# m4drat/wtf

Measured on AMD Instinct MI355X. Metric: execs/sec + emulated instr/s per node (tlv_server, HEVD) at 1/2/4/8 GPUs, higher is better.
Workload: dtype u64

## Files before the change

wtf_amd/csrc/engine.hip:

```cpp
#include <hip/hip_runtime.h>
#include <hipcub/device/device_radix_sort.hpp>

#include <algorithm>
#include <cstddef>
#include <cstdio>
#include <cstdlib>
#include <cstring>
#include <new>
#include <vector>

#include "engine_run.h"
#include "engine_kernels.h"

using namespace wtfgpu_dev;

#define HIPCHK(x)                                                                        \
  do {                                                                                   \
    hipError_t e_ = (x);                                                                 \
    if (e_ != hipSuccess) {                                                              \
      fprintf(stderr, "wtfgpu: %s failed: %s (%s:%d)\n", #x, hipGetErrorString(e_), __FILE__, \
              __LINE__);                                                                 \
      return WTFGPU_ERR_HIP;                                                             \
    }                                                                                    \
  } while (0)
// ... 992 lines not shown
static int set_status_list(wtfgpu_ctx *c, const uint32_t *lanes, uint32_t n, uint32_t status, const uint8_t *skip) {
  if (!c || !c->d_status || (n && !lanes)) return WTFGPU_ERR_INVALID;
  if (n == 0) return WTFGPU_OK;
  for (u32 i = 0; i < n; i++)
    if (lanes[i] >= c->P.nlanes) return WTFGPU_ERR_INVALID;
  HIPCHK(hipSetDevice(c->device));
  const u64 o_skip = ((u64)n * 4 + 255) & ~255ull;
  u8 *st = ring_put(c, nullptr, o_skip + n);
  if (!st || ensure_scratch(c, o_skip + n)) return WTFGPU_ERR_OOM;
  memcpy(st, lanes, (u64)n * 4);
  if (skip) memcpy(st + o_skip, skip, n);
  HIPCHK(hipMemcpyAsync(c->d_scratch, st, skip ? o_skip + n : (u64)n * 4, hipMemcpyHostToDevice, c->stream));
  k_set_status<<<(n + 255) / 256, 256, 0, c->stream>>>(c->P, (const u32 *)c->d_scratch, n, status,
                                                      skip ? c->d_scratch + o_skip : nullptr);
  HIPCHK(hipGetLastError());
  return WTFGPU_OK;
}

int wtfgpu_resume(wtfgpu_ctx *c, const uint32_t *lanes, uint32_t n, const uint8_t *skip_bp) {
  std::vector<u8> zeros;
  if (!skip_bp) {
    zeros.assign(n, 0);
    skip_bp = zeros.data();
  }
  return set_status_list(c, lanes, n, WTFGPU_RUNNING, skip_bp);
}

int wtfgpu_stop(wtfgpu_ctx *c, const uint32_t *lanes, uint32_t n, uint32_t status) {
  return set_status_list(c, lanes, n, status, nullptr);
}

static int regroup_buffers(wtfgpu_ctx *c) {
  if (c->d_rkeys) return WTFGPU_OK;
  const u64 N = c->P.nlanes;
  if (!c->d_perm && dalloc(&c->d_perm, N)) return WTFGPU_ERR_OOM;
  if (dalloc(&c->d_rkeys, N) || dalloc(&c->d_rkeys2, N) || dalloc(&c->d_rlanes, N)) return WTFGPU_ERR_OOM;
  size_t bytes = 0;
  HIPCHK(hipcub::DeviceRadixSort::SortPairs(nullptr, bytes, c->d_rkeys, c->d_rkeys2, c->d_rlanes, c->d_perm, (int)N, 0,
                                            24, c->stream));
  HIPCHK(hipMalloc(&c->d_rtemp, bytes));
  c->rtemp_bytes = bytes;
  return WTFGPU_OK;
}

static Dev run_params(wtfgpu_ctx *c, bool regroup) {
  Dev Q = c->P;
  Q.perm = regroup ? c->d_perm : nullptr;
  Q.stat = c->d_stat;
  const char *w = getenv("WTFGPU_WARM");
  if (!(w && atoi(w) == 0)) {
    const u32 need = (u32)((c->P.nlanes + c->P.lpw - 1) / c->P.lpw);
    if (c->d_warm && c->warm_n < need) {
      (void)hipDeviceSynchronize();
      (void)hipFree(c->d_warm);
      c->d_warm = nullptr;
    }
    if (!c->d_warm) {
      c->warm_n = need;
      const u64 bytes = UC_IMAGE_BYTES * need * UC_QUEUES;
      if (hipMalloc((void **)&c->d_warm, bytes) != hipSuccess) {
        c->d_warm = nullptr;
      } else if (hipMemset(c->d_warm, 0xff, bytes) != hipSuccess || hipDeviceSynchronize() != hipSuccess) {
        (void)hipFree(c->d_warm);
        c->d_warm = nullptr;
      }
    }
    Q.warm = c->d_warm ? c->d_warm + (u64)(c->cur_queue % UC_QUEUES) * UC_IMAGE_BYTES * c->warm_n : nullptr;
    Q.warm_n = c->warm_n;
  } else {
    Q.warm = nullptr;
  }
  return Q;
}

static u64 regroup_now(wtfgpu_ctx *c, u32 count) {
  c->rg_used[c->cur_queue & 1] = 2;
  if (!c->regroup_steps || count < 2 * c->P.lpw) return 0;
  if (!c->regroup_auto) return c->regroup_steps;
  static constexpr double kMargin = 1.1;
  static constexpr u64 kProbe = 32;
  const u64 i = c->rg_runs++;
  bool on;
  if (c->lps_sched[1] == 0) on = true;
  else if (c->lps_sched[0] == 0) on = false;
  else {
    on = c->lps_sched[1] > kMargin * c->lps_sched[0];
    if (i % kProbe == kProbe - 1) on = !on;
  }
  c->rg_used[c->cur_queue & 1] = on;
  return on ? c->regroup_steps : 0;
}
static u64 regroup_now_timed(wtfgpu_ctx *c, u32 count, int &used) {
  used = 2;
  if (!c->regroup_steps || count < 2 * c->P.lpw) return 0;
  if (!c->regroup_auto) return c->regroup_steps;
  static constexpr u64 kProbe = 32;
  const u64 i = c->rg_sync_runs++;
  bool on;
  if (c->nspi_sched[1] == 0) on = true;
  else if (c->nspi_sched[0] == 0) on = false;
  else {
    on = c->nspi_sched[1] < c->nspi_sched[0];
    if (i % kProbe == kProbe - 1) on = !on;
  }
  used = on;
  return on ? c->regroup_steps : 0;
}
static void regroup_observe_timed(wtfgpu_ctx *c, int used, double ms, u64 retired) {
  if (used > 1 || retired < 4096) return;
  const double v = ms * 1e6 / (double)retired;
  double &e = c->nspi_sched[used];
  e = e == 0 ? v : 0.75 * e + 0.25 * v;
}
static void regroup_observe(wtfgpu_ctx *c, u64 group_steps, u64 retired) {
  const u8 used = c->rg_used[c->cur_queue & 1];
  if (used > 1 || group_steps < 64) return;
  const double lps = (double)retired / (double)group_steps;
  double &e = c->lps_sched[used];
  e = e == 0 ? lps : 0.75 * e + 0.25 * lps;
}

static int launch_chunk(wtfgpu_ctx *c, const Dev &Q, u32 first, u32 count, u64 steps, bool regroup) {
  const u32 hwaves = (count + c->P.lpw - 1) / c->P.lpw;
  if (regroup) {
    HIPCHK(hipMemsetAsync(c->d_stat + 2, 0, 16, c->stream));
    k_regroup_keys<<<(count + 255) / 256, 256, 0, c->stream>>>(Q, first, count, c->d_rkeys, c->d_rlanes);
    HIPCHK(hipGetLastError());
    size_t bytes = c->rtemp_bytes;
    HIPCHK(hipcub::DeviceRadixSort::SortPairs(c->d_rtemp, bytes, c->d_rkeys, c->d_rkeys2, c->d_rlanes,
                                              c->d_perm + first, (int)count, 0, 24, c->stream));
  }
  k_run<<<(hwaves + 3) / 4, 256, 0, c->stream>>>(Q, first, count, steps);
  HIPCHK(hipGetLastError());
  return WTFGPU_OK;
}

static void print_stamps(const u64 *s) {
#ifdef WTFGPU_STAMPS
  if (s[0])
    fprintf(stderr,
            "wtfgpu stamps (cycles per wave-step, %llu steps): fast loop %.0f, slow: xlate+fill %.0f, coverage %.0f, "
            "exec %.0f, cross-page %.0f; slow steps: miss %llu, codepage %llu, ucmiss %llu, other %llu; "
            "fast lookup %.0f, fast exec %.0f, bp %.0f\n",
            (unsigned long long)s[0], (double)s[4] / s[0], (double)s[6] / s[0], (double)s[7] / s[0],
            (double)s[5] / s[0], (double)s[9] / s[0], (unsigned long long)s[12], (unsigned long long)s[13],
            (unsigned long long)s[14], (unsigned long long)s[15], (double)s[10] / s[0], (double)s[11] / s[0], (double)s[8] / s[0]);
  fprintf(stderr, "wtfgpu stamps generic ops:");
  for (int k = 0; k < 512; k++)
    if (s[16 + k]) fprintf(stderr, " %d:%llu", k, (unsigned long long)s[16 + k]);
  fprintf(stderr, "\n");
  fprintf(stderr, "wtfgpu stamps bp_apply cycles by kind:");
  for (int k = 0; k < 8; k++) fprintf(stderr, " %d:%llu", k, (unsigned long long)s[528 + k]);
  fprintf(stderr, "\n");
#else
  (void)s;
#endif
}

int wtfgpu_run(wtfgpu_ctx *c, uint32_t first, uint32_t count, uint64_t max_steps, wtfgpu_run_stats_t *stats) {
  if (!lanes_ok(c, first, count) || (first % c->P.lpw)) return WTFGPU_ERR_INVALID;
  if (!c->P.pool) return WTFGPU_ERR_STATE;
  if (c->async_launches) return WTFGPU_ERR_STATE;
  HIPCHK(hipSetDevice(c->device));
  wtfgpu_run_stats_t st{};
  u64 chunk = 1ull << 20;
  const bool to_end = max_steps >= (1ull << 32);
  int used_timed = 2;
  const u64 regroup = to_end ? regroup_now_timed(c, count, used_timed) : regroup_now(c, count);
  if (regroup) {
    chunk = regroup;
    if (int rc = regroup_buffers(c)) return rc;
  }
  const Dev Q = run_params(c, regroup != 0);
  const u32 group = regroup ? (u32)std::max<u64>(1, 4096 / regroup) : 1;
  u64 done = 0;
  float ms_total = 0;
  for (;;) {
    HIPCHK(hipMemsetAsync(c->d_stat, 0, STAT_N * 8, c->stream));
    HIPCHK(hipEventRecord(c->ev0, c->stream));
    u32 k = 0;
    for (; k < group && done < max_steps; k++) {
      const u64 steps = std::min<u64>(chunk, max_steps - done);
      if (int rc = launch_chunk(c, Q, first, count, steps, regroup != 0)) return rc;
      done += steps;
    }
    HIPCHK(hipEventRecord(c->ev1, c->stream));
    u64 s[STAT_N];
    HIPCHK(hipMemcpyAsync(s, c->d_stat, sizeof(s), hipMemcpyDeviceToHost, c->stream));
    HIPCHK(hipStreamSynchronize(c->stream));
    float ms = 0;
    HIPCHK(hipEventElapsedTime(&ms, c->ev0, c->ev1));
    ms_total += ms;
    st.kernel_launches += k;
    st.group_steps += s[0];
    st.lane_retired += s[1];
    print_stamps(s);
    if (s[2] == 0 || done >= max_steps) break;
  }
  if (to_end) regroup_observe_timed(c, used_timed, ms_total, st.lane_retired);
  else regroup_observe(c, st.group_steps, st.lane_retired);
  st.kernel_ms = ms_total;
  if (stats) *stats = st;
  return WTFGPU_OK;
}

int wtfgpu_run_async(wtfgpu_ctx *c, uint32_t first, uint32_t count, uint64_t max_steps) {
  if (!lanes_ok(c, first, count) || (first % c->P.lpw) || max_steps == 0 || max_steps > (1ull << 32))
    return WTFGPU_ERR_INVALID;
  if (!c->P.pool) return WTFGPU_ERR_STATE;
  if (c->async_launches) return WTFGPU_ERR_STATE;
  HIPCHK(hipSetDevice(c->device));
  const u64 regroup = regroup_now(c, count);
  const u64 chunk = regroup ? regroup : max_steps;
  if (regroup)
    if (int rc = regroup_buffers(c)) return rc;
  const Dev Q = run_params(c, regroup != 0);
  HIPCHK(hipEventRecord(c->ev_pre, c->stream));
  c->pre_valid = true;
  HIPCHK(hipMemsetAsync(c->d_stat, 0, STAT_N * 8, c->stream));
  HIPCHK(hipEventRecord(c->ev0, c->stream));
  u32 k = 0;
  for (u64 done = 0; done < max_steps; done += chunk, k++) {
    if (int rc = launch_chunk(c, Q, first, count, std::min<u64>(chunk, max_steps - done), regroup != 0)) return rc;
  }
  HIPCHK(hipEventRecord(c->ev1, c->stream));
  c->async_launches = k;
  return WTFGPU_OK;
}

int wtfgpu_run_wait(wtfgpu_ctx *c, wtfgpu_run_stats_t *stats) {
  if (!c) return WTFGPU_ERR_INVALID;
  wtfgpu_run_stats_t st{};
  if (c->async_launches) {
    HIPCHK(hipSetDevice(c->device));
    u64 s[STAT_N];
    HIPCHK(hipMemcpyAsync(s, c->d_stat, sizeof(s), hipMemcpyDeviceToHost, c->stream));
    HIPCHK(hipStreamSynchronize(c->stream));
    ring_reset(c);
    float ms = 0;
    HIPCHK(hipEventElapsedTime(&ms, c->ev0, c->ev1));
    st.kernel_launches = c->async_launches;
    st.group_steps = s[0];
    st.lane_retired = s[1];
    st.kernel_ms = ms;
    c->async_launches = 0;
    regroup_observe(c, st.group_steps, st.lane_retired);
    print_stamps(s);
  }
  if (stats) *stats = st;
  return WTFGPU_OK;
}

int wtfgpu_prefetch_results(wtfgpu_ctx *c, uint32_t first, uint32_t count, wtfgpu_exit_t *exits, uint64_t *bytes,
                            uint32_t *dirty, uint64_t *stop_args) {
  if (!lanes_ok(c, first, count) || !exits) return WTFGPU_ERR_INVALID;
  if (count == 0) return WTFGPU_OK;
  HIPCHK(hipSetDevice(c->device));
  if (c->exq_cap < count) {
    if (c->d_exq) HIPCHK(hipFreeAsync(c->d_exq, c->stream));
    c->d_exq = nullptr;
    c->exq_cap = 0;
    if (hipMallocAsync((void **)&c->d_exq, (u64)count * sizeof(wtfgpu_exit_t), c->stream) != hipSuccess)
      return WTFGPU_ERR_OOM;
    c->exq_cap = count;
  }
  k_pack_exits<<<(count + 255) / 256, 256, 0, c->stream>>>(c->P, first, count, c->d_exq);
  HIPCHK(hipGetLastError());
  HIPCHK(hipMemcpyAsync(exits, c->d_exq, (u64)count * sizeof(wtfgpu_exit_t), hipMemcpyDeviceToHost, c->stream));
  if (bytes) HIPCHK(hipMemcpyAsync(bytes, c->d_nbytes + first, (u64)count * 8, hipMemcpyDeviceToHost, c->stream));
  if (dirty) HIPCHK(hipMemcpyAsync(dirty, c->d_ovcount + first, (u64)count * 4, hipMemcpyDeviceToHost, c->stream));
  if (stop_args && c->d_stopargs)
    HIPCHK(hipMemcpyAsync(stop_args, c->d_stopargs + (u64)first * 6, (u64)count * 48, hipMemcpyDeviceToHost,
                          c->stream));
  return WTFGPU_OK;
}

constexpr u64 kPcovCap = 1ull << 22;
constexpr u64 kPcovLanes = 256, kPcovRips = kPcovLanes + kPcovCap * 4;

int wtfgpu_prefetch_coverage(wtfgpu_ctx *c, uint32_t first, uint32_t count, uint64_t *hdr) {
  if (!lanes_ok(c, first, count) || !hdr) return WTFGPU_ERR_INVALID;
  if (!c->d_covrip || count == 0) {
    hdr[0] = hdr[1] = 0;
    return WTFGPU_ERR_STATE;
  }
  HIPCHK(hipSetDevice(c->device));
  if (!c->d_pcov && hipMallocAsync((void **)&c->d_pcov, kPcovRips + kPcovCap * 8, c->stream) != hipSuccess) {
    c->d_pcov = nullptr;
    return WTFGPU_ERR_OOM;
  }
  HIPCHK(hipMemsetAsync(c->d_pcov, 0, 16, c->stream));
  k_cov_collect_stopped<<<(count + 3) / 4, 256, 0, c->stream>>>(
      c->P, first, count, (u32 *)(c->d_pcov + kPcovLanes), (u64 *)(c->d_pcov + kPcovRips), kPcovCap,
      (unsigned long long *)c->d_pcov, (u32 *)(c->d_pcov + 8));
  HIPCHK(hipGetLastError());
  HIPCHK(hipMemcpyAsync(hdr, c->d_pcov, 16, hipMemcpyDeviceToHost, c->stream));
  return WTFGPU_OK;
}

int wtfgpu_prefetched_coverage(wtfgpu_ctx *c, uint32_t *out_lanes, uint64_t *out_rips, uint64_t n) {
  if (!c || (n && (!out_lanes || !out_rips)) || n > kPcovCap || (n && !c->d_pcov)) return WTFGPU_ERR_INVALID;
  if (n == 0) return WTFGPU_OK;
  HIPCHK(hipSetDevice(c->device));
  HIPCHK(hipMemcpyAsync(out_lanes, c->d_pcov + kPcovLanes, n * 4, hipMemcpyDeviceToHost, c->stream));
  HIPCHK(hipMemcpyAsync(out_rips, c->d_pcov + kPcovRips, n * 8, hipMemcpyDeviceToHost, c->stream));
  HIPCHK(hipStreamSynchronize(c->stream));
// ... 592 lines not shown
```

wtf_amd/csrc/engine_exec.h:

```cpp
#pragma once
#include "engine_device.h"

namespace wtfgpu_dev {


struct Lane {
  u32 *glo, *ghi;
  u64 rip, rflags, icount, nbytes;
  u64 tv[TLB_N], td[TLB_N];
  u64 bloom;
  u64 cvpn, cptr;
  u64 cr0, cr3, efer;
  u64 exaddr;
  u64 miss_va;
  u32 tnext, ovn, cpl, status, lane, exvec, exerr, exop;
  u32 miss, miss_acc, flush, pend;
  u32 nodeliver;
  u32 cgen, ccnt;
  u32 simd;
};

__device__ __forceinline__ u32 simd_bits(u64 cr0, u64 cr4, u64 xcr0) {
  const bool ts = (cr0 >> 3) & 1;
  const u32 sse = !((cr0 >> 2) & 1) && !ts && ((cr4 >> 9) & 1);
// ... 86 lines not shown
__device__ __forceinline__ void store_le(u8 *p, u32 sz, u64 v) {
  const uintptr_t a = (uintptr_t)p;
  if ((a & (sz - 1)) == 0) {
    if (sz == 8) *(u64 *)p = v;
    else if (sz == 4) *(u32 *)p = (u32)v;
    else if (sz == 2) *(u16 *)p = (u16)v;
    else *p = (u8)v;
    return;
  }
  for (u32 i = 0; i < sz; i++) p[i] = (u8)(v >> (8 * i));
}

enum { ACC_R = 0, ACC_W = 1, ACC_X = 2, ACC_WPROBE = 3 };

__device__ __forceinline__ void set_fault(Lane &L, u32 vec, u32 err, u64 addr) {
  L.status = WTFGPU_EXIT_FAULT;
  L.exvec = vec;
  L.exerr = err;
  L.exaddr = addr;
}

__device__ __forceinline__ bool canonical(u64 va) { return (u64)(((i64)(va << 16)) >> 16) == va; }

__device__ __forceinline__ u32 pf_error(const Lane &L, int acc, bool present) {
  const bool nxe = (L.efer >> 11) & 1;
  return (present ? 1u : 0u) | (acc == ACC_W || acc == ACC_WPROBE ? 2u : 0u) | (L.cpl == 3 ? 4u : 0u) |
         (acc == ACC_X && nxe ? 16u : 0u);
}

__device__ __forceinline__ bool perm_ok(const Lane &L, u64 td, int acc) {
  const bool user = L.cpl == 3;
  const bool wp = (L.cr0 >> 16) & 1;
  const bool w = acc == ACC_W || acc == ACC_WPROBE;
  return !((user && !(td & T_U)) || (w && !(td & T_W) && (user || wp)) || (acc == ACC_X && (td & T_NX)));
}

template <bool kFault = true>
__device__ __forceinline__ bool walk(const Dev &P, Lane &L, u64 va, int acc, u64 &td, u64 &gpfn) {
  const bool nxe = (L.efer >> 11) & 1;
  if (!canonical(va)) {
    if (kFault) set_fault(L, WTFGPU_VEC_GP, 0, va);
    return false;
  }
  u64 table = L.cr3 & 0x000ffffffffff000ull;
  bool aw = true, au = true, nx = false;
  u64 e = 0, pmask = 0xfff;
  bool priv;
  for (int level = 3; level >= 0; level--) {
    const u64 idx = (va >> (12 + 9 * level)) & 0x1ff;
    const u8 *pg = phys_page(P, L.lane, L.ovn, L.bloom, table >> 12, priv);
    e = *(const u64 *)(pg + idx * 8);
    if (!(e & 1)) {
      if (kFault) set_fault(L, WTFGPU_VEC_PF, pf_error(L, acc, false), va);
      return false;
    }
    aw &= (e & 2) != 0;
    au &= (e & 4) != 0;
    if (nxe && (e >> 63)) nx = true;
    if ((level == 2 || level == 1) && (e & 0x80)) {
      pmask = level == 2 ? 0x3fffffffull : 0x1fffffull;
      break;
    }
    table = e & 0x000ffffffffff000ull;
  }
  const u64 gpa = ((e & 0x000ffffffffff000ull) & ~pmask) | (va & pmask);
  gpfn = gpa >> 12;
  const u8 *pg = phys_page(P, L.lane, L.ovn, L.bloom, gpfn, priv);
  td = (u64)(uintptr_t)pg | (aw ? T_W : 0) | (au ? T_U : 0) | (nx ? T_NX : 0) | (priv ? T_PRIV : 0) |
       (is_ptpage(P, gpfn) ? T_PT : 0);
  return true;
}

__device__ __forceinline__ u8 *cow_copy(const Dev &P, u32 lane, u32 slot, u64 gpfn, const u8 *src) {
  u8 *dst = P.ov_data + ((u64)lane * P.K + slot) * WTFGPU_PAGE_SIZE;
  const uint4 *__restrict__ s4 = (const uint4 *)src;
  uint4 *__restrict__ d4 = (uint4 *)dst;
  for (int i = 0; i < 256; i += 16) {
    uint4 t[16];
#pragma unroll
    for (int j = 0; j < 16; j++) t[j] = s4[i + j];
#pragma unroll
    for (int j = 0; j < 16; j++) d4[i + j] = t[j];
  }
  P.ov_gpfn[(u64)slot * P.nlanes + lane] = (u32)gpfn;
  return dst;
}

__device__ __forceinline__ bool service_miss(const Dev &P, Lane &L, u64 va, int acc) {
  u64 td, gpfn;
  if (!walk(P, L, va, acc, td, gpfn)) return false;
  if (!perm_ok(L, td, acc)) {
    set_fault(L, WTFGPU_VEC_PF, pf_error(L, acc, true), va);
    return false;
  }
  if (acc == ACC_W && !(td & T_PRIV)) {
    if (L.ovn >= P.K) {
      L.status = WTFGPU_EXIT_OVERLAY_FULL;
      return false;
    }
    u8 *np = cow_copy(P, L.lane, L.ovn, gpfn, (const u8 *)(uintptr_t)(td & ~0xfffull));
    L.ovn++;
    L.bloom |= bloom_bit(gpfn);
    tlb_flush(L);
    td = (u64)(uintptr_t)np | (td & 0xfff) | T_PRIV;
  }
  tlb_put(L, va >> 12, td);
  return true;
}

__device__ __forceinline__ bool fast_fill(const Dev &P, Lane &L) {
  const u64 va = L.miss_va;
  const int acc = (int)L.miss_acc;
  u64 td, gpfn;
  if (!walk<false>(P, L, va, acc, td, gpfn) || !perm_ok(L, td, acc)) return false;
  if (acc == ACC_W && !(td & T_PRIV)) {
    if ((td & T_PT) || L.ovn >= P.K) return false;
    u8 *np = cow_copy(P, L.lane, L.ovn, gpfn, (const u8 *)(uintptr_t)(td & ~0xfffull));
    L.ovn++;
    L.bloom |= bloom_bit(gpfn);
    tlb_flush(L);
    td = (u64)(uintptr_t)np | (td & 0xfff) | T_PRIV;
  }
  tlb_put(L, va >> 12, td);
  return true;
}

__device__ __forceinline__ bool fast_fill_prep(const Dev &P, Lane &L, u64 &src, u64 &dst, u64 &gpfn, u64 &td) {
  const u64 va = L.miss_va;
  const int acc = (int)L.miss_acc;
  dst = 0;
  if (!walk<false>(P, L, va, acc, td, gpfn) || !perm_ok(L, td, acc)) return false;
  if (acc == ACC_W && !(td & T_PRIV)) {
    if ((td & T_PT) || L.ovn >= P.K) return false;
    src = td & ~0xfffull;
    dst = (u64)(uintptr_t)(P.ov_data + ((u64)L.lane * P.K + L.ovn) * WTFGPU_PAGE_SIZE);
    return true;
  }
  tlb_put(L, va >> 12, td);
  return true;
}
__device__ __forceinline__ void fast_fault(const Dev &P, Lane &L) {
  const u64 va = L.miss_va;
  const int acc = (int)L.miss_acc;
  u64 td, gpfn;
  if (!walk(P, L, va, acc, td, gpfn)) return;
  if (!perm_ok(L, td, acc)) set_fault(L, WTFGPU_VEC_PF, pf_error(L, acc, true), va);
}
__device__ __forceinline__ void fast_fill_finish(const Dev &P, Lane &L, u64 dst, u64 gpfn, u64 td) {
  P.ov_gpfn[(u64)L.ovn * P.nlanes + L.lane] = (u32)gpfn;
  L.ovn++;
  L.bloom |= bloom_bit(gpfn);
  tlb_flush(L);
  tlb_put(L, L.miss_va >> 12, dst | (td & 0xfff) | T_PRIV);
}

__device__ __forceinline__ u8 *xlate(Lane &L, u64 va, int acc, u64 *tdo = nullptr) {
  u64 td;
  if (!tlb_get(L, va >> 12, td)) {
    L.miss = 1;
    L.miss_va = va;
    L.miss_acc = (u32)acc;
    return nullptr;
  }
  if (!perm_ok(L, td, acc)) {
    set_fault(L, WTFGPU_VEC_PF, pf_error(L, acc, true), va);
    return nullptr;
  }
  if (acc == ACC_W && !(td & T_PRIV)) {
    L.miss = 1;
    L.miss_va = va;
    L.miss_acc = (u32)acc;
    return nullptr;
  }
  if (tdo) *tdo = td;
  return (u8 *)(uintptr_t)(td & ~0xfffull) + (va & 0xfff);
}

__device__ __forceinline__ bool span_w(Lane &L, u64 va, u32 n) {
  const u64 last = (va + n - 1) & ~0xfffull;
  const bool two = ((va ^ (va + n - 1)) >> 12) != 0;
  if (!xlate(L, va, ACC_WPROBE) || (two && !xlate(L, last, ACC_WPROBE))) return false;
  return xlate(L, va, ACC_W) && (!two || xlate(L, last, ACC_W));
}

struct TenetDev {
  u8 *buf;
  u64 cap;
  u64 *pos, *cpos, *ipos, *last;
  u32 *mute;
};
__device__ TenetDev g_tn;
enum : u32 { TN_R = 1, TN_W = 2, TN_RW = 3 };
constexpr u64 TN_ACC = 1ull << 56, TN_REGS = 2ull << 56;

__device__ __noinline__ void tn_access(u32 lane, u64 va, u32 len, u32 type) {
  if (g_tn.mute[lane]) return;
  const u64 p = g_tn.pos[lane], last = g_tn.last[lane];
  u8 *const base = g_tn.buf + (u64)lane * g_tn.cap;
  if (type == TN_W && last != ~0ull && last + 16 <= g_tn.cap && *(const u64 *)(base + last) == va &&
      *(const u64 *)(base + last + 8) == (TN_ACC | (u64)TN_RW << 32 | len))
    return;
  const u64 n = 16 + ((u64)len + 7) / 8 * 8;
  if (p + n <= g_tn.cap) {
    *(u64 *)(base + p) = va;
    *(u64 *)(base + p + 8) = TN_ACC | (u64)type << 32 | len;
  } else if (p + 16 <= g_tn.cap) {
    *(u64 *)(base + p) = 0;
    *(u64 *)(base + p + 8) = 0;
  }
  g_tn.last[lane] = p;
  g_tn.pos[lane] = p + n;
}
__device__ __forceinline__ void tn_mute(u32 lane) {
  if (g_tn.buf) g_tn.mute[lane]++;
}
__device__ __forceinline__ bool tn_unmute(u32 lane, u64 va, u32 len, u32 type, bool ok) {
  if (g_tn.buf) {
    g_tn.mute[lane]--;
    if (ok) tn_access(lane, va, len, type);
  }
  return ok;
}
__device__ __forceinline__ void tn_insn_begin(u32 lane) {
  if (!g_tn.buf) return;
  g_tn.ipos[lane] = g_tn.cpos[lane] = g_tn.pos[lane];
  g_tn.last[lane] = ~0ull;
  g_tn.mute[lane] = 0;
}
__device__ __forceinline__ void tn_rollback(u32 lane) {
  if (!g_tn.buf) return;
  g_tn.pos[lane] = g_tn.cpos[lane];
  g_tn.last[lane] = ~0ull;
  g_tn.mute[lane] = 0;
}
__device__ __forceinline__ void tn_commit(u32 lane) {
  if (g_tn.buf) g_tn.cpos[lane] = g_tn.pos[lane];
}

__device__ __forceinline__ bool vread(Lane &L, u64 va, u32 sz, u64 &out, int acc = ACC_R) {
  const u32 off = (u32)(va & 0xfff);
  if (off + sz <= 4096) {
    const u8 *p = xlate(L, va, acc);
    if (!p) return false;
    out = load_le(p, sz);
  } else {
    const u32 n0 = 4096 - off;
    if (acc == ACC_W) {
      if (!xlate(L, va, ACC_WPROBE) || !xlate(L, va + n0, ACC_WPROBE)) return false;
    }
    const u8 *p0 = xlate(L, va, acc);
    if (!p0) return false;
    const u8 *p1 = xlate(L, va + n0, acc);
    if (!p1) return false;
    u64 v = 0;
    for (u32 i = 0; i < sz; i++) v |= (u64)(i < n0 ? p0[i] : p1[i - n0]) << (8 * i);
    out = v;
  }
  L.pend += sz;
  if (g_tn.buf) tn_access(L.lane, va, sz, acc == ACC_W ? TN_RW : TN_R);
  return true;
}

__device__ __forceinline__ bool vwrite(Lane &L, u64 va, u32 sz, u64 v) {
  const u32 off = (u32)(va & 0xfff);
  u64 td0 = 0, td1 = 0;
  if (off + sz <= 4096) {
    u8 *p = xlate(L, va, ACC_W, &td0);
    if (!p) return false;
    store_le(p, sz, v);
  } else {
    const u32 n0 = 4096 - off;
    if (!xlate(L, va, ACC_WPROBE) || !xlate(L, va + n0, ACC_WPROBE)) return false;
    u8 *p0 = xlate(L, va, ACC_W, &td0);
    if (!p0) return false;
    u8 *p1 = xlate(L, va + n0, ACC_W, &td1);
    if (!p1) return false;
    for (u32 i = 0; i < sz; i++) {
      if (i < n0) p0[i] = (u8)(v >> (8 * i));
      else p1[i - n0] = (u8)(v >> (8 * i));
    }
  }
  if ((td0 | td1) & T_PT) L.flush = 1;
  L.pend += sz;
  if (g_tn.buf) tn_access(L.lane, va, sz, TN_W);
  return true;
}

__device__ __noinline__ void tn_regs(const Dev &P, Lane &L) {
  const u32 lane = L.lane;
  const u64 cap = g_tn.cap, end = g_tn.pos[lane];
  u8 *const base = g_tn.buf + (u64)lane * cap;
  const u32 st = L.status, ev = L.exvec, ee = L.exerr, cpl = L.cpl, pend = L.pend, miss = L.miss;
  const u64 ea = L.exaddr, cr0 = L.cr0;
  L.cpl = 0;
  L.cr0 &= ~(1ull << 16);
  for (u64 q = g_tn.ipos[lane]; q + 16 <= end && q + 16 <= cap;) {
    const u64 va = *(const u64 *)(base + q), meta = *(const u64 *)(base + q + 8);
    if (meta >> 56 != 1) break;
    const u32 len = (u32)(meta & 0xffffffffull);
    const u64 n = 16 + ((u64)len + 7) / 8 * 8;
    if (q + n > cap) break;
    {
      u8 *out = base + q + 16;
      for (u32 i = 0; i < len; i++) {
        u8 b = 0;
        for (int attempt = 0;; attempt++) {
// ... 31 lines not shown
```

wtf_amd/csrc/engine_run.h:

```cpp
#pragma once
#include <hip/hip_runtime.h>

#include "engine_fast.h"

using namespace wtfgpu_dev;

namespace {

__device__ __forceinline__ u64 wave_sum(u64 v) {
#pragma unroll
  for (int off = 32; off > 0; off >>= 1) v += __shfl_xor(v, off, 64);
  return v;
}
__device__ __forceinline__ u64 readlane64(u64 v, int l) {
  const u32 lo = __builtin_amdgcn_readlane((u32)v, l);
  const u32 hi = __builtin_amdgcn_readlane((u32)(v >> 32), l);
  return ((u64)hi << 32) | lo;
}
__device__ __forceinline__ u64 m_eq32(u32 a, u32 b) { return __builtin_amdgcn_uicmp(a, b, 32); }
__device__ __forceinline__ u64 m_ne32(u32 a, u32 b) { return __builtin_amdgcn_uicmp(a, b, 33); }
__device__ __forceinline__ u64 m_eq64(u64 a, u64 b) { return __builtin_amdgcn_uicmpl(a, b, 32); }
__device__ __forceinline__ u64 m_ne64(u64 a, u64 b) { return __builtin_amdgcn_uicmpl(a, b, 33); }
__device__ __forceinline__ u64 m_lt64(u64 a, u64 b) { return __builtin_amdgcn_uicmpl(a, b, 36); }
__device__ __forceinline__ u64 m_ge64(u64 a, u64 b) { return __builtin_amdgcn_uicmpl(a, b, 35); }
// ... 758 lines not shown
        term = ((c >> (8 * (b & 7))) & 0xff) == 0;
      }
      if (term) break;
    }
  }
  const u64 rsp = R(L, WTFGPU_RSP);
  u64 ra = 0;
  for (int attempt = 0;; attempt++) {
    L.miss = 0;
    if (vread(L, rsp, 8, ra)) break;
    if (L.status != WTFGPU_RUNNING || !L.miss || !miss_service(P, L, attempt)) {
      L.status = WTFGPU_RUNNING;
      L.miss = 0;
      L.pend = 0;
      return false;
    }
  }
  L.pend = 0;
  RS(L, WTFGPU_RAX, a.value);
  RS(L, WTFGPU_RSP, rsp + 8);
  L.rip = ra;
  return true;
}

__device__ __noinline__ bool bp_apply(const Dev &P, Lane &L, u64 grip, const wtfgpu_bp_action_t *found = nullptr) {
  tn_mute(L.lane);
  const bool r = bp_apply_action(P, L, grip, found);
  tn_unmute(L.lane, 0, 0, 0, false);
  return r;
}

__device__ __noinline__ void slow_step(const Dev &P, Lane &L, u64 grip, u64 lptr, bool ing, bool &skip) {
  const u32 off = (u32)(grip & 0xfff);
  const bool m32 = (lptr & EFER_M32) != 0;
  lptr &= ~EFER_M32;
  IBytes ib;
  ib.avail = 4096 - off < 16 ? 4096 - off : 16;
  fetch_bytes(lptr, off, ib.avail, ib.lo, ib.hi);
  UOp d;
  int dr = decode(ib, d, m32);
  if (dr == 1) {
    u64 nptr = 0;
    if (ing) {
      const u64 va2 = (grip & ~0xfffull) + 4096;
      u64 td;
      if (!tlb_get(L, va2 >> 12, td) || !perm_ok(L, td, ACC_X)) {
        if (service_miss(P, L, va2, ACC_X)) tlb_get(L, va2 >> 12, td);
        else td = 0;
      }
      if (td) nptr = td & ~0xfffull;
      else ing = false;
    }
    const u64 cm = __ballot(ing);
    if (cm == 0) return;
    const int leader = __ffsll((long long)cm) - 1;
    const u64 lnptr = readlane64(nptr, leader);
    ing = ing && nptr == lnptr;
    const u32 n0 = ib.avail;
    u64 lo2, hi2;
    fetch_bytes(lnptr, 0, 16 - n0, lo2, hi2);
    if (n0 >= 8) {
      ib.hi = (n0 == 8 ? 0 : ib.hi) | (n0 == 8 ? lo2 : (lo2 << (8 * (n0 - 8))));
    } else {
      ib.lo = ib.lo | (lo2 << (8 * n0));
      ib.hi = (lo2 >> (64 - 8 * n0)) | (hi2 << (8 * n0));
    }
    ib.avail = 16;
    dr = decode(ib, d, m32);
  }
  if (dr == 2) {
    if (ing) set_fault(L, WTFGPU_VEC_GP, 0, 0);
    return;
  }
  const u64 gmask = __ballot(ing);
  if (gmask == 0) return;
  if (P.cov_rip) L.ccnt = cover(P, grip, ing, L.lane, L.cgen, L.ccnt);
  if (P.trace && ing && !skip) trace_rip(P, L.lane, grip);
  const bool isbp = bp_lookup(P, grip);
  if (ing) {
    if (isbp && !skip) {
      const bool applied = bp_apply(P, L, grip);
      if (!applied) L.status = WTFGPU_EXIT_BREAKPOINT;
      skip = applied && L.rip == grip;
      if (applied && !skip && g_tn.buf) tn_regs(P, L);
      ing = false;
    } else {
      skip = false;
    }
  }
  if (!d.supported) {
    if (ing) {
      L.status = WTFGPU_EXIT_UNIMPLEMENTED;
      L.exop = d.len >= 4 ? d.opbytes : (d.opbytes & ((1u << (8 * d.len)) - 1));
    }
    return;
  }
  if (ing) {
    u64 next = 0;
    int x;
    tn_insn_begin(L.lane);
    for (int attempt = 0;; attempt++) {
      L.miss = 0;
      L.pend = 0;
      tn_rollback(L.lane);
      x = exec(P, L, d, grip + d.len, next);
      if (!L.miss || L.status != WTFGPU_RUNNING) break;
      if (!miss_service(P, L, attempt)) break;
    }
    retire(P, L, x, d.len, next, d.opbytes);
    if (g_tn.buf && (x == X_OK || x == X_CR3)) tn_regs(P, L);
    if (P.edges && P.cov_rip && edge_op(d.op, d.bsrc) && x == X_OK) {
      const u32 c0 = L.ccnt;
      L.ccnt = cover_edge(P, edge_key(grip, next), true, L.lane, L.cgen, L.ccnt);
      count_edge(P, L.lane, L.ccnt != c0);
    }
  }
}

struct LaneCopy {
  Lane l;
  u32 r[32];
};
#define WITH_LANE_COPY(call)                      \
  do {                                            \
    LaneCopy &C_ = ((LaneCopy *)P.lcopy)[lane];   \
    Lane &T = C_.l;                               \
    u32 *const tlo_ = C_.r, *const thi_ = C_.r + 16; \
    _Pragma("unroll") for (int i_ = 0; i_ < 16; i_++) { \
      tlo_[i_] = glo[i_];                         \
      thi_[i_] = ghi[i_];                         \
    }                                             \
    T = L;                                        \
    T.glo = tlo_;                                 \
    T.ghi = thi_;                                 \
    call;                                         \
    L = T;                                        \
    L.glo = glo;                                  \
    L.ghi = ghi;                                  \
    _Pragma("unroll") for (int i_ = 0; i_ < 16; i_++) { \
      glo[i_] = tlo_[i_];                         \
      ghi[i_] = thi_[i_];                         \
    }                                             \
  } while (0)

#ifdef WTFGPU_STAMPS
#define STAMP(k)                                   \
  do {                                             \
    const u64 t_ = __builtin_amdgcn_s_memtime();   \
    stamp_[k] += t_ - tprev_;                      \
    tprev_ = t_;                                   \
  } while (0)
#define WHY(k) why_ = (k)
#define OPHIST(op) ophist_[((op) & 63) | (why_ & 3) << 6 | ((op) & 64 ? 256 : 0)]++
constexpr u32 STAT_N = 536;
#else
constexpr u32 STAT_N = 16;
#define OPHIST(op) \
  do {             \
  } while (0)
#define STAMP(k) \
  do {           \
  } while (0)
#define WHY(k) \
  do {         \
  } while (0)
#endif

#define RECONVERGE() __builtin_amdgcn_wave_barrier()

constexpr u32 FILL_PREFETCH = 8;
__global__ __launch_bounds__(256, 2) void k_run(Dev P, u32 first, u32 count, u64 max_steps) {
  if (P.perm && rfl64(P.stat[3]) == 0) return;
  const u32 lid = threadIdx.x & 63;
  const u32 hw = rfl32(blockIdx.x * 4 + (threadIdx.x >> 6));
  const u32 tid = hw * P.lpw + lid;
  const bool inrange = lid < P.lpw && tid < count && first + tid < P.nlanes;
  const u32 lane = inrange ? (P.perm ? P.perm[first + tid] : first + tid) : 0;
  const bool valid = inrange && P.status[lane] == WTFGPU_RUNNING;
  __shared__ UCEntry sUC[4][UC_N];
  __shared__ UCUop sUU[4][UC_U];
  UCEntry *uc = sUC[threadIdx.x >> 6];
  UCUop *uu = sUU[threadIdx.x >> 6];
  const bool wave_live = __ballot(valid) != 0;
  const UCEntry *img = (P.warm && wave_live) ? (const UCEntry *)P.warm + (u64)(hw % P.warm_n) * UC_N : nullptr;
  if (img) {
    for (u32 i = lid; i < UC_N; i += 64) {
      UCEntry t = img[i];
      t.logged = 0;
      if (P.cov_rip && t.key != EMPTY_KEY && !(t.flags & (UC_COVERED | UC_CROSS | UC_BADLEN)))
        t.flags |= covered_flag_lane(P, t.rip, (u32)(t.rip & 0xfff));
      uc[i] = t;
    }
  } else {
    for (u32 i = lid; i < UC_N; i += 64) uc[i].key = EMPTY_KEY;
  }
  if (lid < UC_U) uu[lid].key = EMPTY_KEY;
  u32 glo[16], ghi[16];
  Lane L;
  L.glo = glo;
  L.ghi = ghi;
  if (valid) {
    load_lane(P, lane, L);
  } else {
    L.status = WTFGPU_EXIT_IDLE;
    L.lane = 0;
    L.rip = 0;
    L.icount = 0;
    L.cvpn = EMPTY_KEY;
  }
  const u64 icount0 = L.icount;
  bool skip = valid && (P.lflags[lane] & 1);
  if (valid && g_tn.buf && (g_tn.pos[lane] == 0 || (P.lflags[lane] & 2))) WITH_LANE_COPY(tn_regs(P, T));
  const bool cov_on = rfl32(P.cov_rip != nullptr ? 1u : 0u) != 0;
  u64 pool_lo = (u64)(uintptr_t)P.pool, pool_span = (P.npool + 1) * WTFGPU_PAGE_SIZE;
  u64 limit_v = P.limit ? P.limit : ~0ull;
  u32 max32 = max_steps > 0xffffffffull ? 0xffffffffu : (u32)max_steps;
  asm volatile("" : "+v"(pool_lo), "+v"(pool_span), "+v"(limit_v), "+v"(max32));
  const FastMem fm = fast_mem(P);
  u32 steps = 0;
#ifdef WTFGPU_STAMPS
  u64 stamp_[8] = {0, 0, 0, 0, 0, 0, 0, 0};
  u64 tprev_ = __builtin_amdgcn_s_memtime();
  u64 whyc_[4] = {0, 0, 0, 0};
  u32 why_ = 3;
  u32 ophist_[512] = {};
  u64 bpcyc_[8] = {};
#endif

  for (;;) {
    u64 grip = 0;
    bool have = false;
    for (;;) {
      if (m_ge32(steps, max32)) break;
      const u64 am = m_eq32(L.status, WTFGPU_RUNNING);
      if (am == 0) break;
      grip = readlane64(L.rip, __ffsll((long long)am) - 1);
      u64 gm = am & m_eq64(L.rip, grip);
      if (gm != am) {
        for (u64 lo = am & m_lt64(L.rip, grip); lo; lo = am & m_lt64(L.rip, grip))
          grip = readlane64(L.rip, __ffsll((long long)lo) - 1);
        gm = am & m_eq64(L.rip, grip);
      }
      have = true;
      WHY(1);
      if (const u64 cxm = gm & m_ne64(L.cvpn, grip >> 12)) {
        if (in_mask(cxm)) {
          u64 td, gp;
          bool ok = tlb_get(L, grip >> 12, td) && perm_ok(L, td, ACC_X);
          if (!ok && walk<false>(P, L, grip & ~0xfffull, ACC_X, td, gp) && perm_ok(L, td, ACC_X)) {
            tlb_put(L, grip >> 12, td);
            ok = true;
          }
          if (ok) {
            L.cvpn = grip >> 12;
            L.cptr = (td & ~0xfffull) | (L.efer & EFER_M32);
          }
        }
        if (gm & m_ne64(L.cvpn, grip >> 12)) break;
      }
      WHY(3);
      const u64 lptr = readlane64(L.cptr, __ffsll((long long)gm) - 1);
      if (m_ge64(lptr - pool_lo, pool_span)) break;
      const u64 ingm = gm & m_eq64(L.cptr, lptr);
      const bool ing = in_mask(ingm);
      const u64 key = lptr | (grip & 0xfff);
      UCEntry *e = &uc[uc_slot(key)];
      UCHead h;
      uc_head_read(e, h);
      if (h.key != key) uc_head_read(++e, h);
      WHY(2);
      if (h.key != key) break;
      WHY(3);
      const u32 flags = h.flags;
      if (flags & (UC_CROSS | UC_BADLEN | UC_UNSUP)) break;
      if ((flags & UC_BP) && (ingm & ~__ballot(skip))) break;
      if (cov_on && !(flags & UC_COVERED) && (ingm & ~rfl64(e->logged))) break;
      const FOp &f = h.f;
      if (fo_op(f) == FO_GENERIC) break;
      if (!(f.fl & (FF_PUSH | FF_POP | FF_MR_A | FF_MR_B | FF_MW)) && fo_op(f) < FO_VLD) {
        steps++;
        have = false;
        if (ing) {
          skip = false;
          const u32 len = fo_len(f);
          FOp fr = f;
          asm volatile("" : "+s"(fr.w0), "+s"(fr.fl), "+s"(fr.w2), "+s"(fr.disp), "+s"(fr.imm));
          u64 next;
          fast_exec<true>(fm, L, fr, grip + len, next);
          L.rip = next;
          L.icount++;
          L.nbytes += len;
          if (L.icount > limit_v) L.status = WTFGPU_EXIT_TIMEOUT;
        }
        RECONVERGE();
        continue;
      }
      steps++;
      have = false;
      STAMP(6);
      const u32 len = fo_len(f);
      u64 next = 0;
      u64 wantm = ingm;
      if (ing) skip = false;
      for (u32 round = 0;; round++) {
        if (in_mask(wantm)) {
          L.miss = 0;
          L.pend = 0;
          FOp fr = f;
          asm volatile("" : "+s"(fr.w0), "+s"(fr.fl), "+s"(fr.w2), "+s"(fr.disp), "+s"(fr.imm));
          fast_exec(fm, L, fr, grip + len, next);
        }
        RECONVERGE();
        wantm = round >= 3 ? 0 : wantm & m_eq32(L.miss, 2);
        if (wantm == 0) break;
        u64 csrc = 0, cdst = 0, cgpfn = 0, ctd = 0;
        bool want = in_mask(wantm);
        if (want && !fast_fill_prep(P, L, csrc, cdst, cgpfn, ctd)) {
          want = false;
          fast_fault(P, L);
        }
        for (u64 cm = __ballot(want && cdst); cm; cm &= cm - 1) {
          const int l = __ffsll((long long)cm) - 1;
          const uint4 *s4 = (const uint4 *)(uintptr_t)readlane64(csrc, l) + lid * 4;
          uint4 *d4 = (uint4 *)(uintptr_t)readlane64(cdst, l) + lid * 4;
          const uint4 a = s4[0], b = s4[1], c = s4[2], d = s4[3];
          d4[0] = a;
          d4[1] = b;
          d4[2] = c;
          d4[3] = d;
        }
        __builtin_amdgcn_fence(__ATOMIC_ACQ_REL, "workgroup");
        if (want && cdst) fast_fill_finish(P, L, cdst, cgpfn, ctd);
        wantm = __ballot(want);
      }
      const u64 missm = ingm & m_ne32(L.miss, 0);
      if (in_mask(ingm & ~missm)) {
        L.rip = next;
        L.icount++;
        L.nbytes += len + L.pend;
        if (L.icount > limit_v) L.status = WTFGPU_EXIT_TIMEOUT;
      }
      RECONVERGE();
      STAMP(7);
      if (missm & m_eq32(L.status, WTFGPU_RUNNING)) {
        WHY(0);
        steps--;
        have = true;
        break;
      }
      if (missm) break;
    }
    STAMP(0);
    if (__ballot(L.status == WTFGPU_EXIT_FAULT && !L.nodeliver)) {
      if (L.status == WTFGPU_EXIT_FAULT && !L.nodeliver) {
        bool dv;
        WITH_LANE_COPY(dv = deliver_fault(P, T));
        if (dv && g_tn.buf) WITH_LANE_COPY(tn_regs(P, T));
      }
      RECONVERGE();
      continue;
    }
    if (!have) break;

    steps++;
#ifdef WTFGPU_STAMPS
    whyc_[why_ & 3]++;
#endif
    const bool active = L.status == WTFGPU_RUNNING;
    bool cand = active && L.rip == grip;
    if (cand && (grip >> 12) != L.cvpn) WITH_LANE_COPY(code_xlate(P, T, grip));
    cand = cand && (grip >> 12) == L.cvpn;
    const u64 cm = __ballot(cand);
    if (cm == 0) continue;
    const int leader = __ffsll((long long)cm) - 1;
    const u64 lptr = readlane64(L.cptr, leader);
    bool ing = cand && L.cptr == lptr;

    const u32 off = (u32)(grip & 0xfff);
    const u64 key = lptr | off;
    UCEntry *e = &uc[uc_slot(key)];
    if (rfl64(e->key) != key) {
      if (rfl64(e[1].key) == key) e += 1;
      else if (cacheable_key(lptr, pool_lo, pool_span)) {
        if (lid < 16) ((u32 *)&e[1])[lid] = ((const u32 *)e)[lid];
        __builtin_amdgcn_wave_barrier();
      }
    }
    const bool cacheable = !m_ge64(lptr - pool_lo, pool_span);
    if (cacheable && rfl64(e->key) != key) {
      if (!uc_fill_shared(P, e, &uu[uu_slot(key)], key, off, grip, lid))
        uc_fill(P, e, &uu[uu_slot(key)], key, lptr, off, grip, lid, true);
      const UCEntry *pe = e;
      u64 prip = grip;
      for (u32 k = 0; k < FILL_PREFETCH; k++) {
        const u32 pf = rfl32(pe->flags), pw0 = rfl32(pe->f.w0), plen = (pw0 >> 20) & 0x3f;
        if ((pf & (UC_CROSS | UC_BADLEN)) || !plen) break;
        const u64 nxt = prip + plen;
        if ((nxt >> 12) != (grip >> 12) || (nxt & 0xfff) > 4096 - 16) break;
        const u32 poff = (u32)(nxt & 0xfff);
        const u64 pkey = lptr | poff;
        UCEntry *ps = &uc[uc_slot(pkey)];
        if (rfl64(ps->key) == pkey || rfl64(ps[1].key) == pkey) break;
        if (!uc_fill_shared(P, ps + 1, nullptr, pkey, poff, nxt, lid)) break;
        pe = ps + 1;
        prip = nxt;
      }
      const u32 ff = rfl32(e->flags);
      if (!(ff & (UC_BP | UC_CROSS | UC_BADLEN | UC_UNSUP)) && (!cov_on || (ff & UC_COVERED)) &&
          (rfl32(e->f.w0) & 0xff) != FO_GENERIC) {
        steps--;
        STAMP(2);
        continue;
      }
    }
    STAMP(2);
    const u32 flags = cacheable ? rfl32(e->flags) : UC_CROSS;
    if (flags & (UC_CROSS | UC_BADLEN)) {
      if (flags & UC_BADLEN) {
        if (ing) set_fault(L, WTFGPU_VEC_GP, 0, 0);
      } else if (L.status != WTFGPU_EXIT_IDLE) {
        bool sk = skip;
        WITH_LANE_COPY(slow_step(P, T, grip, lptr, ing, sk));
        skip = sk;
      }
      RECONVERGE();
      STAMP(5);
      continue;
    }
    const u32 len = (rfl32(e->f.w0) >> 20) & 0x3f;
    const u64 gmask = __ballot(ing);

    if (P.trace && ing && !skip) trace_rip(P, L.lane, grip);
    bool logged_now = false;
    if (cov_on && !(flags & UC_COVERED)) {
      const u64 logged = rfl64(e->logged);
      if (gmask & ~logged) {
        L.ccnt = cover(P, grip, ing && !((logged >> lid) & 1), L.lane, L.cgen, L.ccnt);
        if (lid == 0) e->logged = logged | gmask;
        logged_now = true;
      }
    }
    STAMP(3);
    if (logged_now && !(flags & (UC_BP | UC_UNSUP)) && (rfl32(e->f.w0) & 0xff) != FO_GENERIC) {
      steps--;
      continue;
    }
    u32 act_kind = ~0u;
    const wtfgpu_bp_action_t *act = nullptr;
    if ((flags & UC_BP) && P.act_keys && !g_tn.buf) {
      u32 slot;
      if (hash_find(P.act_keys, P.act_mask, grip, slot)) {
        act = &P.act[slot];
        act_kind = rfl32(act->kind);
      }
    }
#ifdef WTFGPU_STAMPS
    if (__ballot(ing && (flags & UC_BP) && !skip)) OPHIST(56 + (act_kind < 7 ? act_kind : 7));
#endif
    if (act_kind == WTFGPU_BPACT_SET_GPRS && ing && !skip) {
#pragma unroll
      for (u32 i = 0; i < 16; i++) RS(L, i, act->gprs[i]);
      L.rip = act->gprs[16];
      skip = L.rip == grip;
      ing = false;
    }
    if (act_kind == WTFGPU_BPACT_STOP_OK && ing && !skip) {
      L.status = WTFGPU_EXIT_STOP_OK;
      skip = true;
      ing = false;
    }
    if (act_kind == WTFGPU_BPACT_FEED && P.feed_pos) {
      bool want = false;
      if (ing && !skip) {
        const u64 pos = P.feed_pos[L.lane];
        const u64 end = P.feed_end[L.lane];
        if (pos != ~0ull && pos + 4 <= end) {
          const u8 *src = P.feed_data + pos;
          const u32 n = (u32)src[0] | ((u32)src[1] << 8) | ((u32)src[2] << 16) | ((u32)src[3] << 24);
          const u64 win = act->value;
          if (n && n < win && pos + 4 + n <= end) {
            const u64 va = R(L, (u32)act->gprs[0] & 15) + win - n;
            u64 td;
            if (!(tlb_get(L, va >> 12, td) && (td & T_PRIV))) {
              L.miss_va = va;
              L.miss_acc = ACC_W;
              want = true;
            }
          }
        }
      }
      u64 csrc = 0, cdst = 0, cgpfn = 0, ctd = 0;
      if (want) {
        const u32 cpl0 = L.cpl;
        const u64 cr00 = L.cr0;
        L.cpl = 0;
        L.cr0 &= ~(1ull << 16);
        want = fast_fill_prep(P, L, csrc, cdst, cgpfn, ctd);
        L.cpl = cpl0;
        L.cr0 = cr00;
      }
      RECONVERGE();
      for (u64 cm = __ballot(want && cdst); cm; cm &= cm - 1) {
        const int l = __ffsll((long long)cm) - 1;
        const uint4 *s4 = (const uint4 *)(uintptr_t)readlane64(csrc, l) + lid * 4;
        uint4 *d4 = (uint4 *)(uintptr_t)readlane64(cdst, l) + lid * 4;
        const uint4 a = s4[0], b = s4[1], c = s4[2], d = s4[3];
        d4[0] = a;
        d4[1] = b;
        d4[2] = c;
        d4[3] = d;
      }
      __builtin_amdgcn_fence(__ATOMIC_ACQ_REL, "workgroup");
      if (want && cdst) fast_fill_finish(P, L, cdst, cgpfn, ctd);
      RECONVERGE();
    }
    if (ing) {
      if ((flags & UC_BP) && !skip) {
        bool applied = false;
#ifdef WTFGPU_STAMPS
        const u64 tb_ = __builtin_amdgcn_s_memtime();
#endif
        if (P.act_keys) WITH_LANE_COPY(applied = bp_apply(P, T, grip, act));
#ifdef WTFGPU_STAMPS
        bpcyc_[act_kind < 7 ? act_kind : 7] += __builtin_amdgcn_s_memtime() - tb_;
#endif
        if (!applied) L.status = WTFGPU_EXIT_BREAKPOINT;
        skip = applied && L.rip == grip;
        if (applied && !skip && g_tn.buf) WITH_LANE_COPY(tn_regs(P, T));
        ing = false;
      } else {
        skip = false;
      }
    }
    STAMP(4);
    const UOp *u = nullptr;
    if (__ballot(ing)) u = uc_uop(P, uu, key, lptr, off, grip, lid);
    if (__ballot(ing) && !(flags & UC_UNSUP)) OPHIST(rfl32(u->op) + (flags & UC_COVERED ? 64 : 0));
    if (ing && (flags & UC_UNSUP)) {
      const u32 ob = u->opbytes, n = len;
      L.status = WTFGPU_EXIT_UNIMPLEMENTED;
      L.exop = n >= 4 ? ob : (ob & ((1u << (8 * n)) - 1));
      ing = false;
    }
    if (ing) {
      u64 next = 0;
      int x;
      WITH_LANE_COPY(x = exec_retry(P, T, u, next));
      u32 opbytes = 0;
      if (x == X_UNIMPL) opbytes = u->opbytes;
      retire(P, L, x, len, next, opbytes);
      if (g_tn.buf && (x == X_OK || x == X_CR3)) WITH_LANE_COPY(tn_regs(P, T));
      if (P.edges && P.cov_rip && x == X_OK && edge_op(rfl32(u->op), rfl32(u->bsrc))) {
        const u32 c0 = L.ccnt;
        L.ccnt = cover_edge(P, edge_key(grip, next), true, L.lane, L.cgen, L.ccnt);
        count_edge(P, L.lane, L.ccnt != c0);
      }
    }
    RECONVERGE();
    STAMP(1);
  }

  if (P.warm && wave_live && hw < P.warm_n) {
    __builtin_amdgcn_wave_barrier();
    __builtin_amdgcn_fence(__ATOMIC_ACQUIRE, "wavefront");
    UCEntry *out = (UCEntry *)P.warm + (u64)hw * UC_N;
    for (u32 i = lid; i < UC_N; i += 64) out[i] = uc[i];
  }
  if (valid && g_tn.buf && L.status != WTFGPU_RUNNING && L.status != WTFGPU_EXIT_BREAKPOINT &&
      g_tn.pos[lane] > g_tn.ipos[lane])
    WITH_LANE_COPY(tn_regs(P, T));
  if (valid) {
    store_lane(P, L);
    store_tlb(P, L);
    if (L.status == WTFGPU_EXIT_FAULT || L.status == WTFGPU_EXIT_UNIMPLEMENTED) {
      ExitInfo ei;
      ei.vector = L.exvec;
      ei.error = L.exerr;
      ei.opcode = L.exop;
      ei.cpl = L.cpl;
      ei.addr = L.exaddr;
      P.exinfo[lane] = ei;
    }
    P.lflags[lane] = skip ? 1u : 0u;
  }
  const u64 retired = wave_sum(valid ? L.icount - icount0 : 0);
  const u64 running = wave_sum((valid && L.status == WTFGPU_RUNNING) ? 1 : 0);
  if (lid == 0) {
    atomicAdd((unsigned long long *)&P.stat[0], (unsigned long long)steps);
    atomicAdd((unsigned long long *)&P.stat[1], (unsigned long long)retired);
    if (running) atomicAdd((unsigned long long *)&P.stat[2], (unsigned long long)running);
#ifdef WTFGPU_STAMPS
    for (int k = 0; k < 8; k++) atomicAdd((unsigned long long *)&P.stat[4 + k], (unsigned long long)stamp_[k]);
    for (int k = 0; k < 4; k++) atomicAdd((unsigned long long *)&P.stat[12 + k], (unsigned long long)whyc_[k]);
    for (int k = 0; k < 512; k++)
      if (ophist_[k]) atomicAdd((unsigned long long *)&P.stat[16 + k], (unsigned long long)ophist_[k]);
    for (int k = 0; k < 8; k++) atomicAdd((unsigned long long *)&P.stat[528 + k], (unsigned long long)bpcyc_[k]);
#endif
  }
}

}
```

Measured before the change: 15.89 million.

## Handle return and feed breakpoint actions inline in the fast loop

Adds in-kernel handling of RETURN breakpoint actions. It scans the string argument for a terminator through a read-only page walk, then pops the return address and sets RAX. It also completes FEED actions (stop or copy into a writable private page) directly in the run loop instead of deferring to bp_apply. The aim is to avoid the heavier generic bp_apply path, with its lane copy, for the common breakpoint kinds. In exchange it adds divergent code, new noinline helpers and extra reconvergence points, and it duplicates semantics that must match bp_apply exactly.

```diff
diff --git a/wtf_amd/csrc/engine.hip b/wtf_amd/csrc/engine.hip
--- a/wtf_amd/csrc/engine.hip
+++ b/wtf_amd/csrc/engine.hip
@@ -1168,6 +1168,9 @@
   fprintf(stderr, "wtfgpu stamps bp_apply cycles by kind:");
   for (int k = 0; k < 8; k++) fprintf(stderr, " %d:%llu", k, (unsigned long long)s[528 + k]);
   fprintf(stderr, "\n");
+  fprintf(stderr, "wtfgpu stamps bp hits in registers / left to bp_apply (lanes): return %llu / %llu, feed %llu / %llu\n",
+          (unsigned long long)s[536], (unsigned long long)s[537], (unsigned long long)s[538],
+          (unsigned long long)s[539]);
 #else
   (void)s;
 #endif
diff --git a/wtf_amd/csrc/engine_exec.h b/wtf_amd/csrc/engine_exec.h
--- a/wtf_amd/csrc/engine_exec.h
+++ b/wtf_amd/csrc/engine_exec.h
@@ -262,6 +262,58 @@
   L.bloom |= bloom_bit(gpfn);
   tlb_flush(L);
   tlb_put(L, L.miss_va >> 12, dst | (td & 0xfff) | T_PRIV);
+}
+
+__device__ __noinline__ u64 walk_read(const Dev &P, u64 va, u64 cr3, u64 efer, u64 bloom, u32 lane, u32 ovn) {
+  Lane T;
+  T.cr3 = cr3;
+  T.efer = efer;
+  T.bloom = bloom;
+  T.lane = lane;
+  T.ovn = ovn;
+  u64 td, gpfn;
+  return walk<false>(P, T, va, ACC_R, td, gpfn) ? td : 0;
+}
+
+__device__ __forceinline__ u64 read_xlate(const Dev &P, Lane &L, u64 va) {
+  u64 td;
+  if (tlb_get(L, va >> 12, td)) return perm_ok(L, td, ACC_R) ? td : 0;
+  td = walk_read(P, va, L.cr3, L.efer, L.bloom, L.lane, L.ovn);
+  if (!td || !perm_ok(L, td, ACC_R)) return 0;
+  tlb_put(L, va >> 12, td);
+  return td;
+}
+
+__device__ __noinline__ void feed_copy(u8 *__restrict__ d, const u8 *__restrict__ sp, u32 n) {
+  u32 k = 0;
+  for (; k + 32 <= n; k += 32) {
+    u8 t[32];
+#pragma unroll
+    for (u32 j = 0; j < 32; j++) t[j] = sp[k + j];
+#pragma unroll
+    for (u32 j = 0; j < 32; j++) d[k + j] = t[j];
+  }
+  if (k < n) {
+    u8 t[32];
+#pragma unroll
+    for (u32 j = 0; j < 32; j++) t[j] = k + j < n ? sp[k + j] : 0;
+#pragma unroll
+    for (u32 j = 0; j < 32; j++)
+      if (k + j < n) d[k + j] = t[j];
+  }
+}
+
+__device__ __noinline__ bool block_has_zero(const u64 *w, u32 from, u32 to) {
+  const u64 c[4] = {w[0], w[1], w[2], w[3]};
+  u32 pos = 32;
+#pragma unroll
+  for (int k = 3; k >= 0; k--) {
+    const u32 sk = from > 8u * k ? from - 8u * k : 0;
+    const u64 v = c[k] | (sk >= 8 ? ~0ull : (1ull << (8 * sk)) - 1);
+    const u64 z = (v - 0x0101010101010101ull) & ~v & 0x8080808080808080ull;
+    if (z) pos = 8u * k + ((u32)__builtin_ctzll(z) >> 3);
+  }
+  return pos < to;
 }
 
 __device__ __forceinline__ u8 *xlate(Lane &L, u64 va, int acc, u64 *tdo = nullptr) {
diff --git a/wtf_amd/csrc/engine_run.h b/wtf_amd/csrc/engine_run.h
--- a/wtf_amd/csrc/engine_run.h
+++ b/wtf_amd/csrc/engine_run.h
@@ -934,7 +934,7 @@
   } while (0)
 #define WHY(k) why_ = (k)
 #define OPHIST(op) ophist_[((op) & 63) | (why_ & 3) << 6 | ((op) & 64 ? 256 : 0)]++
-constexpr u32 STAT_N = 536;
+constexpr u32 STAT_N = 540;
 #else
 constexpr u32 STAT_N = 16;
 #define OPHIST(op) \
@@ -1007,6 +1007,7 @@
   u32 why_ = 3;
   u32 ophist_[512] = {};
   u64 bpcyc_[8] = {};
+  u32 bpin_[4] = {0, 0, 0, 0};
 #endif
 
   for (;;) {
@@ -1251,17 +1252,64 @@
       skip = true;
       ing = false;
     }
+    if (act_kind == WTFGPU_BPACT_RETURN && ing && !skip) {
+      const u64 rsp = R(L, WTFGPU_RSP);
+      bool ok = (rsp & 0xfff) <= 4096 - 8;
+      u64 ra = 0;
+      const u32 sreg = rfl32((u32)act->gprs[0]);
+      if (ok && sreg) {
+        const u64 s = R(L, (sreg - 1) & 15), lim = act->gprs[1];
+        for (u64 i = 0; i < lim;) {
+          const u64 va = s + i, al = va & ~31ull;
+          const u64 td = read_xlate(P, L, al);
+          if (!td || (td & T_PT)) {
+            ok = false;
+            break;
+          }
+          const u64 *w = (const u64 *)(uintptr_t)((td & ~0xfffull) + (al & 0xfff));
+          const u32 b = (u32)(va - al);
+          const u64 room = 32 - b, m = lim - i < room ? lim - i : room;
+          if (block_has_zero(w, b, b + (u32)m)) break;
+          i += m;
+        }
+      }
+      if (ok) {
+        const u64 td = read_xlate(P, L, rsp);
+        ok = td && !(td & T_PT);
+        if (ok) ra = load_le((const u8 *)(uintptr_t)(td & ~0xfffull) + (rsp & 0xfff), 8);
+      }
+#ifdef WTFGPU_STAMPS
+      bpin_[ok ? 0 : 1]++;
+#endif
+      if (ok) {
+        RS(L, WTFGPU_RAX, act->value);
+        RS(L, WTFGPU_RSP, rsp + 8);
+        L.rip = ra;
+        L.pend = 0;
+        L.miss = 0;
+        skip = L.rip == grip;
+        ing = false;
+      }
+    }
+    RECONVERGE();
     if (act_kind == WTFGPU_BPACT_FEED && P.feed_pos) {
-      bool want = false;
+      bool want = false, fstop = false, fcopy = false;
+      u64 fpos = 0;
+      u32 fn = 0;
       if (ing && !skip) {
         const u64 pos = P.feed_pos[L.lane];
         const u64 end = P.feed_end[L.lane];
+        if (pos != ~0ull && pos + 4 > end) fstop = true;
         if (pos != ~0ull && pos + 4 <= end) {
           const u8 *src = P.feed_data + pos;
           const u32 n = (u32)src[0] | ((u32)src[1] << 8) | ((u32)src[2] << 16) | ((u32)src[3] << 24);
           const u64 win = act->value;
+          fpos = pos + 4;
+          fn = n;
+          if (n >= win || pos + 4 + n > end) fstop = true;
           if (n && n < win && pos + 4 + n <= end) {
-            const u64 va = R(L, (u32)act->gprs[0] & 15) + win - n;
+            const u64 va = R(L, rfl32((u32)act->gprs[0]) & 15) + win - n;
+            fcopy = true;
             u64 td;
             if (!(tlb_get(L, va >> 12, td) && (td & T_PRIV))) {
               L.miss_va = va;
@@ -1294,6 +1342,30 @@
       }
       __builtin_amdgcn_fence(__ATOMIC_ACQ_REL, "workgroup");
       if (want && cdst) fast_fill_finish(P, L, cdst, cgpfn, ctd);
+      RECONVERGE();
+      const u64 fdst = R(L, rfl32((u32)act->gprs[0]) & 15) + act->value - fn;
+      u64 ftd = 0;
+      fcopy = fcopy && ((fdst ^ (fdst + fn - 1)) >> 12) == 0 && tlb_get(L, fdst >> 12, ftd) &&
+              (ftd & (T_PRIV | T_PT)) == T_PRIV;
+#ifdef WTFGPU_STAMPS
+      if (ing && !skip) bpin_[fstop || fcopy ? 2 : 3]++;
+#endif
+      if (fstop) {
+        if (fpos) P.feed_pos[L.lane] = fpos + fn;
+        L.status = WTFGPU_EXIT_STOP_OK;
+        skip = true;
+        ing = false;
+      }
+      if (fcopy) {
+        feed_copy((u8 *)(uintptr_t)(ftd & ~0xfffull) + (fdst & 0xfff), P.feed_data + fpos, fn);
+        P.feed_pos[L.lane] = fpos + fn;
+        RS(L, rfl32((u32)act->gprs[1]) & 15, fn);
+        RS(L, rfl32((u32)act->gprs[0]) & 15, fdst);
+        L.pend = 0;
+        L.miss = 0;
+        skip = true;
+        ing = false;
+      }
       RECONVERGE();
     }
     if (ing) {
@@ -1367,6 +1439,10 @@
   }
   const u64 retired = wave_sum(valid ? L.icount - icount0 : 0);
   const u64 running = wave_sum((valid && L.status == WTFGPU_RUNNING) ? 1 : 0);
+#ifdef WTFGPU_STAMPS
+  u64 bpins_[4];
+  for (int k = 0; k < 4; k++) bpins_[k] = wave_sum(bpin_[k]);
+#endif
   if (lid == 0) {
     atomicAdd((unsigned long long *)&P.stat[0], (unsigned long long)steps);
     atomicAdd((unsigned long long *)&P.stat[1], (unsigned long long)retired);
@@ -1377,6 +1453,7 @@
     for (int k = 0; k < 512; k++)
       if (ophist_[k]) atomicAdd((unsigned long long *)&P.stat[16 + k], (unsigned long long)ophist_[k]);
     for (int k = 0; k < 8; k++) atomicAdd((unsigned long long *)&P.stat[528 + k], (unsigned long long)bpcyc_[k]);
+    for (int k = 0; k < 4; k++) atomicAdd((unsigned long long *)&P.stat[536 + k], (unsigned long long)bpins_[k]);
 #endif
   }
 }
```

Result: faster. 16.75 million, median of 6 (+5.4%).
